# mitroitskii/crosscoder-model-diff-replication

Measured on AMD Instinct MI355X. Metric: activations/sec per train step (fwd+bwd+Adam), 2x2304->16384; % bf16 MFMA peak, higher is better.
Workload: dtype bf16; 1 GPU; crosscoder train step 2x2304->16384, batch 4096; global_batch=4096, n_models=2, d_model=2304, dict_size=16384, parallelism=latent1

## Files before the change

crosscoder-model-diff-replication_amd/csrc/gemm.hip:

```cpp
#include <mutex>

#include <hip/hip_ext.h>

#include "cc_common.h"

namespace cc {

#include "grad_tail.h"
#include "loss_tail.h"

constexpr int BM = 256, NTHR = 512;
constexpr uint32_t OOB = 0x7ffffff0u;
constexpr uint32_t MAX_RECORDS = 0x7fffffe0u;

enum Epi { EPI_F32 = 0, EPI_ENC = 1, EPI_DEC = 2, EPI_DACTS = 3, EPI_WGDEC = 4, EPI_WGENC = 5, EPI_SPLIT = 6, EPI_DLOSS = 7 };

struct GemmArgs {
  const void* A;
  const void* B;
  int64_t lda, ldb;
  int M, N, K;
  int nbm, nbn;
  void* out;
  int64_t ldo;
// ... 392 lines not shown
    const char* la = smem + (kt % NST) * STAGE;
    const char* lb = la + A_BYTES;
    if constexpr (!SPREAD) {
#pragma unroll
      for (int q = 0; q < D; ++q) dma(q, nxt, snx, pf);
    }
    if constexpr (DT == CC_BF16) {
      constexpr int KB = 1;
#pragma unroll
      for (int k0 = 0; k0 < KK; k0 += KB) {
        bf16x8 a[KB][WG::TM], b[KB][WG::TN];
#pragma unroll
        for (int u = 0; u < KB; ++u) {
#pragma unroll
          for (int j = 0; j < WG::TN; ++j) {
            const int c0 = wc * WG::WTN + j * 16;
            b[u][j] = BKC ? frag_kc_bf16<KROW>(lb, c0, k0 + u, lane) : frag_mn_bf16_at<BNT, KROW>(lb, offB[j], k0 + u);
          }
#pragma unroll
          for (int i = 0; i < WG::TM; ++i) {
            const int r0 = wr * WG::WTM + i * 16;
            a[u][i] = AKC ? frag_kc_bf16<KROW>(la, r0, k0 + u, lane) : frag_mn_bf16_at<BM, KROW>(la, offA[i], k0 + u);
          }
        }
        if (SPREAD && k0 == 0) {
#pragma unroll
          for (int q = 0; q < D; ++q) dma(q, nxt, snx, pf);
        }
#pragma unroll
        for (int u = 0; u < KB; ++u)
#pragma unroll
          for (int i = 0; i < WG::TM; ++i)
#pragma unroll
            for (int j = 0; j < WG::TN; ++j)
              acc[i][j] = __builtin_amdgcn_mfma_f32_16x16x32_bf16(b[u][j], a[u][i], acc[i][j], 0, 0, 0);
        __builtin_amdgcn_sched_group_barrier(0x100, KB * (WG::TM * (AKC ? 1 : 2) + WG::TN * (BKC ? 1 : 2)), 0);
        __builtin_amdgcn_sched_group_barrier(0x008, KB * WG::TM * WG::TN, 0);
      }
    } else {
#pragma unroll
      for (int kk = 0; kk < KK; ++kk) {
        f32x4 b[WG::TN];
#pragma unroll
        for (int j = 0; j < WG::TN; ++j) {
          const int c0 = wc * WG::WTN + j * 16;
          b[j] = BKC ? frag_kc_f32<KROW>(lb, c0, kk, lane) : frag_mn_f32_at<BNT, KROW>(lb, offB[j], kk);
        }
#pragma unroll
        for (int i = 0; i < WG::TM; ++i) {
          if (SPREAD && kk == 0) {
#pragma unroll
            for (int q = 0; q < D; ++q)
              if (q * WG::TM / D == i) dma(q, nxt, snx, pf);
          }
          const int r0 = wr * WG::WTM + i * 16;
          f32x4 a = AKC ? frag_kc_f32<KROW>(la, r0, kk, lane) : frag_mn_f32_at<BM, KROW>(la, offA[i], kk);
#pragma unroll
          for (int e = 0; e < 4; ++e)
#pragma unroll
            for (int j = 0; j < WG::TN; ++j)
              acc[i][j] = __builtin_amdgcn_mfma_f32_16x16x4f32(b[j][e], a[e], acc[i][j], 0, 0, 0);
        }
      }
    }
  }
  wait_vmcnt<0>();

  gemm_epilogue<DT, EPI, BNT>(args, acc, tm, m0, n0, wr, wc, lane, blockIdx.x * 8 + wave);
}

#include "gemm_pp.h"
#include "gemm_q4_tile.h"

constexpr int CC_WGRAD_CLOCK_WORDS = 8;
struct WgradTail {
  RedSeg red[2];
  int red_blocks[2];
  ClipArgs clip;
  unsigned* counter;
  float* tile_sum;
  uint64_t* clock;
};

template <bool AKC, bool BKC, int EPI0, int EPI1>
__global__ __launch_bounds__(NTHR, 1) void gemm_pp_dual_tail_kernel(const GemmArgs a0, const GemmArgs a1,
                                                                   const WgradTail tl) {
  __shared__ __attribute__((aligned(16))) char smem[EPI0 == EPI_WGDEC || EPI1 == EPI_WGDEC ? PP_LDS_W : PP_LDS];
  const uint64_t clk0 = __builtin_amdgcn_s_memtime(), wall0 = __builtin_amdgcn_s_memrealtime();
  {
    const int grp = threadIdx.x >> 8, t = threadIdx.x & 255;
    float(*red)[RED_COLS] = (float(*)[RED_COLS])(smem + grp * 4 * RED_COLS * sizeof(float));
    const int nred = tl.red_blocks[0] + tl.red_blocks[1];
    for (int base = 2 * (int)blockIdx.x; base < nred; base += 2 * (int)gridDim.x) {
      const int b = base + grp;
      const int role = b < tl.red_blocks[0] ? 0 : 1, rb = role ? b - tl.red_blocks[0] : b;
      if (b < nred) reduce_rows_phase1(tl.red[role], rb, t, red);
      __syncthreads();
      if (b < nred) reduce_rows_phase2<CC_BF16>(tl.red[role], rb, t, red);
      __syncthreads();
    }
  }
  const int nb0 = a0.nbm * a0.nbn;
  float* wsum_lds = (float*)(smem + PP_SLOT + 64);
  const int wave = threadIdx.x >> 6;
  for (TileLoop L(2 * nb0, a0.tile_ctr, a0.wave_sync); L.more();) {
    const int t = L.begin();
    const int tid = pp_opaque_tid();
    float w;
    if (t < nb0) w = pp_tile<AKC, BKC, EPI0>(a0, smem, t, tid);
    else w = pp_tile<AKC, BKC, EPI1>(a1, smem, t - nb0, tid);
    pp_tile_boundary();
    if ((threadIdx.x & 63) == 0) wsum_lds[wave] = w;
    L.advance(smem);
    if (!L.ctr) __syncthreads();
    if (threadIdx.x == 0) {
      float s = 0.f;
#pragma unroll
      for (int k = 0; k < 8; ++k) s += wsum_lds[k];
      tl.tile_sum[t] = s;
    }
  }
  __builtin_amdgcn_s_waitcnt(0);
  __syncthreads();
  int* last = (int*)smem;
  if (threadIdx.x == 0) {
    __builtin_amdgcn_fence(__ATOMIC_RELEASE, "agent");
    const bool is_last = atomicAdd(tl.counter, 1u) == gridDim.x - 1;
    if (is_last) __builtin_amdgcn_fence(__ATOMIC_ACQUIRE, "agent");
    *last = is_last;
  }
  __syncthreads();
  if (!*last) return;
  {
    double s[8] = {0, 0, 0, 0, 0, 0, 0, 0};
    for (int k = threadIdx.x; k < nb0; k += NTHR) s[1] += (double)tl.tile_sum[k];
    for (int k = threadIdx.x; k < nb0; k += NTHR) s[0] += (double)tl.tile_sum[nb0 + k];
    for (int k = threadIdx.x; k < tl.red_blocks[0]; k += NTHR) s[2] += (double)tl.red[0].sq_part[k];
    for (int k = threadIdx.x; k < tl.red_blocks[1]; k += NTHR) s[3] += (double)tl.red[1].sq_part[k];
    clip_finish<NTHR>(tl.clip, s, (double(*)[NTHR / 64])(smem + 64),
                      (float*)(smem + 64 + 8 * (NTHR / 64) * sizeof(double)));
  }
  if (threadIdx.x == 0) {
    atomicExch(tl.counter, 0u);
    const uint64_t clk1 = __builtin_amdgcn_s_memtime(), wall1 = __builtin_amdgcn_s_memrealtime();
    if (tl.clock) {
      tl.clock[0] += clk1 - clk0;
      tl.clock[1] += wall1 - wall0;
      tl.clock[2] += 1;
    }
  }
}

#ifndef CC_Q4_MASK
#define CC_Q4_MASK 2
#endif
#ifdef CC_DEBUG_HOOKS
static int g_pp_mask = 7, g_pp_fast = 1, g_dec_one_launch = 1, g_q4 = CC_Q4_MASK;
#define CC_DEBUG_API extern "C" __attribute__((visibility("default")))
CC_DEBUG_API void cc_debug_set_q4(int mask) { g_q4 = mask; }
CC_DEBUG_API int cc_debug_get_q4() { return CC_Q4_MASK; }
CC_DEBUG_API void cc_debug_set_pp_mask(int mask) { g_pp_mask = mask; }
CC_DEBUG_API void cc_debug_set_pp_fast(int on) { g_pp_fast = on; }
CC_DEBUG_API void cc_debug_set_dec_one_launch(int on) { g_dec_one_launch = on; }
static int g_wave_sync = 0;
static uint64_t* g_stamps = nullptr;
CC_DEBUG_API void cc_debug_set_stamps(void* buf) { g_stamps = (uint64_t*)buf; }
static int g_epi_store = 1;
CC_DEBUG_API void cc_debug_set_epi_store(int on) { g_epi_store = on; }
static void debug_epi_store(GemmArgs& a, int64_t stamp_tile0 = 0) {
  if (!g_epi_store) a.out = a.out_t = nullptr;
  if (g_stamps) a.stamps = g_stamps + stamp_tile0 * 12;
}
CC_DEBUG_API void cc_debug_set_wave_sync(int on) { g_wave_sync = on; }
static void debug_wave_sync(GemmArgs& a, hipStream_t st) {
  static uint32_t* words = nullptr;
  if (!g_wave_sync) return;
  if (!words && hipMalloc((void**)&words, 64) != hipSuccess) return;
  if (hipMemsetAsync(words, 0, 32, st) != hipSuccess) return;
  a.wave_sync = words;
  a.tile_ctr = nullptr;
}
__global__ __launch_bounds__(NTHR) void debug_spin_kernel(int64_t ticks) {
  extern __shared__ char hold[];
  const uint64_t t0 = wall_clock64();
  if (threadIdx.x == 0) hold[0] = 0;
  while (wall_clock64() - t0 < (uint64_t)ticks) __builtin_amdgcn_s_sleep(8);
}
CC_DEBUG_API int cc_debug_spin(int64_t blocks, int64_t lds_bytes, int64_t ns, void* stream) {
  if (blocks <= 0 || blocks > 4096 || lds_bytes < 0 || lds_bytes > 160 * 1024 || ns < 0 || ns > 1000000000)
    return CC_ERR_SHAPE;
  if (lds_bytes > 65536 && hipFuncSetAttribute((const void*)debug_spin_kernel,
                                               hipFuncAttributeMaxDynamicSharedMemorySize, (int)lds_bytes) != hipSuccess)
    return CC_ERR_SHAPE;
  hipLaunchKernelGGL(debug_spin_kernel, dim3((unsigned)blocks), dim3(NTHR), (unsigned)lds_bytes, (hipStream_t)stream,
                     (int64_t)(ns / 10));
  CC_LAUNCH_CHECK();
  return CC_OK;
}
CC_DEBUG_API int cc_debug_spin_ev(int64_t blocks, int64_t ns, void* stream, void* stop_event) {
  if (blocks <= 0 || blocks > 4096 || ns < 0 || ns > 1000000000) return CC_ERR_SHAPE;
  hipExtLaunchKernelGGL(debug_spin_kernel, dim3((unsigned)blocks), dim3(NTHR), 0, (hipStream_t)stream, nullptr,
                        (hipEvent_t)stop_event, 0, (int64_t)(ns / 10));
  CC_LAUNCH_CHECK();
  return CC_OK;
}
#else
constexpr int g_pp_mask = 7, g_pp_fast = 1, g_dec_one_launch = 1, g_q4 = CC_Q4_MASK;
#endif
static bool use_pp(int64_t N, bool akc, bool bkc, int dtype) {
  if (dtype != CC_BF16 || (!akc && bkc) || N % 8) return false;
  const int bit = akc && bkc ? 0 : (akc ? 1 : 2);
  return (g_pp_mask >> bit) & 1;
}
static int set_pre(GemmArgs& a, const cc_colsum_job* job) {
  if (!job) return CC_OK;
  if (!job->part || !job->out) return CC_ERR_NULL;
  if (job->rows <= 0 || job->cols <= 0 || job->ld < job->cols) return CC_ERR_SHAPE;
  a.pre = {job->part, (int)job->rows, (int)job->cols, job->ld, job->scale, job->out, nullptr, nullptr, nullptr, nullptr};
  a.pre_blocks = (int)((job->cols + RED_COLS - 1) / RED_COLS);
  return CC_OK;
}

static int set_tail(GemmArgs& a, const cc_loss_tail_job* j) {
  if (!j) return CC_OK;
  if (!j->colsum_acts || !j->tn || !j->l1_part || !j->row_part || !j->scalars || !j->counter) return CC_ERR_NULL;
  if (j->h <= 0 || j->B <= 0 || j->n <= 0 || j->ncb <= 0) return CC_ERR_SHAPE;
  a.tail = make_loss_tail_args(j->colsum_acts, j->tn, j->h, j->l1_part, j->row_part, j->ncb, j->l0_part, j->n_l0, j->ev,
                               j->ev_a, j->ev_b, j->scalars, j->l1l0_out, j->host_out, j->seq, j->B, j->n, j->counter);
  a.tail_items = a.tail.l1_wgs + a.tail.ev.nblk;
  return CC_OK;
}

extern "C" int cc_transposed_ok(int64_t B, int64_t K, int64_t h, int dtype) {
  return dtype == CC_BF16 && B % 8 == 0 && K % 8 == 0 && h % 8 == 0 && use_pp(h, true, true, dtype) &&
         use_pp(K, true, true, dtype);
}
static int pick_bn(int64_t N, bool akc, bool bkc, int dtype) {
  if (use_pp(N, akc, bkc, dtype)) return 256;
  return (!bkc && dtype == CC_BF16 && N % 288 == 0) ? 288 : 256;
}
static int64_t n_blocks(int64_t M, int64_t N, int bn) { return ((M + BM - 1) / BM) * ((N + bn - 1) / bn); }

template <int DT, bool AKC, bool BKC, int EPI, int BNT>
static int launch(GemmArgs a, hipStream_t st) {
  a.nbm = (a.M + BM - 1) / BM;
  a.nbn = (a.N + BNT - 1) / BNT;
  dim3 grid(a.nbm * a.nbn), block(NTHR);
  hipLaunchKernelGGL((gemm_kernel<DT, AKC, BKC, EPI, BNT>), grid, block, 0, st, a);
  CC_LAUNCH_CHECK();
  return CC_OK;
}

static int pp_grid(int64_t tiles) {
  static int cus = 0;
  static std::once_flag once;
  std::call_once(once, [] {
    int dev = 0, n = 0;
    if (hipGetDevice(&dev) == hipSuccess && hipDeviceGetAttribute(&n, hipDeviceAttributeMultiprocessorCount, dev) ==
                                                 hipSuccess && n > 0)
      cus = n;
    else
      cus = 256;
  });
  return (int)(tiles < cus ? tiles : cus);
}

template <bool AKC, bool BKC, int EPI>
static int launch_pp(GemmArgs a, hipStream_t st) {
#ifdef CC_DEBUG_HOOKS
  debug_epi_store(a);
#endif
  a.nbm = (a.M + BM - 1) / BM;
  a.nbn = (a.N + 255) / 256;
  if constexpr (EPI == EPI_ENC || EPI == EPI_DACTS) {
    if (g_pp_fast && a.M % BM == 0 && a.N % 256 == 0 &&
        (EPI == EPI_DACTS ? a.mask_bits != nullptr : a.flag && !a.wave_part0)) {
      if constexpr (AKC && BKC) {
        if ((g_q4 >> (EPI == EPI_ENC ? 0 : 1)) & 1 && a.K % 64 == 0 && a.K >= 128 && a.lda == a.ldb) {
          if constexpr (EPI == EPI_ENC)
            hipLaunchKernelGGL((gemm_q4_enc_kernel<true>), dim3(pp_grid(a.nbm * a.nbn)), dim3(Q4_THREADS), 0, st, a);
          else
            hipLaunchKernelGGL((gemm_q4_kernel<EPI, true>), dim3(pp_grid(a.nbm * a.nbn)), dim3(Q4_THREADS), 0, st, a);
          CC_LAUNCH_CHECK();
          return CC_OK;
        }
      }
      hipLaunchKernelGGL((gemm_pp_kernel<AKC, BKC, EPI, true>), dim3(pp_grid(a.nbm * a.nbn)), dim3(NTHR), 0, st, a);
      CC_LAUNCH_CHECK();
      return CC_OK;
    }
  }
  hipLaunchKernelGGL((gemm_pp_kernel<AKC, BKC, EPI>), dim3(pp_grid(a.nbm * a.nbn)), dim3(NTHR), 0, st, a);
  CC_LAUNCH_CHECK();
  return CC_OK;
}

template <int EPI, bool AKC, bool BKC>
static int launch_dt(int dtype, GemmArgs a, hipStream_t st) {
  if constexpr (!(!AKC && BKC)) {
    if (use_pp(a.N, AKC, BKC, dtype)) return launch_pp<AKC, BKC, EPI>(a, st);
  }
  if constexpr (!BKC) {
    if (pick_bn(a.N, AKC, BKC, dtype) == 288) return launch<CC_BF16, AKC, BKC, EPI, 288>(a, st);
  }
  if (dtype == CC_BF16) return launch<CC_BF16, AKC, BKC, EPI, 256>(a, st);
  if (dtype == CC_F32) return launch<CC_F32, AKC, BKC, EPI, 256>(a, st);
  return CC_ERR_DTYPE;
}

static bool al16(const void* p) { return ((uintptr_t)p & 15) == 0; }

static int check_gemm(const GemmArgs& a, int dtype, bool akc, bool bkc) {
  if (!a.A || !a.B) return CC_ERR_NULL;
  if (dtype != CC_BF16 && dtype != CC_F32) return CC_ERR_DTYPE;
  if (a.M <= 0 || a.N <= 0 || a.K <= 0) return CC_ERR_SHAPE;
  int epc = dtype == CC_BF16 ? 8 : 4;
  if (akc && (a.K % epc)) return CC_ERR_SHAPE;
  if (!akc && (a.M % epc)) return CC_ERR_SHAPE;
  if (bkc && (a.K % epc)) return CC_ERR_SHAPE;
  if (!bkc && (a.N % epc)) return CC_ERR_SHAPE;
  if (a.N % 4 || a.ldo % 4) return CC_ERR_SHAPE;
  if ((a.lda % epc) || (a.ldb % epc)) return CC_ERR_ALIGN;
  if (!al16(a.A) || !al16(a.B)) return CC_ERR_ALIGN;
  int es = dtype == CC_BF16 ? 2 : 4;
  uint64_t ra = akc ? (uint64_t)BM * a.lda * es : (uint64_t)a.K * a.lda * es;
  uint64_t rb = bkc ? (uint64_t)288 * a.ldb * es : (uint64_t)a.K * a.ldb * es;
  if (ra >= MAX_RECORDS || rb >= MAX_RECORDS) return CC_ERR_TOO_LARGE;
  return CC_OK;
}

}

using namespace cc;

extern "C" {

int64_t cc_col_part_rows(int64_t M) { return 2 * ((M + BM - 1) / BM); }
int64_t cc_wave_parts(int64_t M, int64_t N) { return 8 * n_blocks(M, N, 256); }
int64_t cc_wgrad_parts(int64_t h, int64_t K, int dtype) { return 8 * n_blocks(h, K, pick_bn(K, false, false, dtype)); }
int64_t cc_wgrad_tile_sums(int64_t h, int64_t K) { return 2 * n_blocks(h, K, 256) + CC_WGRAD_CLOCK_WORDS; }

int cc_gemm_f32out(const void* A, int a_layout, int64_t lda, const void* Bm, int b_layout, int64_t ldb, float* C,
                   int64_t ldc, int64_t M, int64_t N, int64_t K, int dtype, void* stream) {
  GemmArgs a = {};
  a.A = A; a.B = Bm; a.lda = lda; a.ldb = ldb; a.M = (int)M; a.N = (int)N; a.K = (int)K;
  a.out = C; a.ldo = ldc;
  if (!C) return CC_ERR_NULL;
  if (((uintptr_t)C & 15) != 0) return CC_ERR_ALIGN;
  bool akc = a_layout == CC_LAYOUT_KC, bkc = b_layout == CC_LAYOUT_KC;
  int rc = check_gemm(a, dtype, akc, bkc);
  if (rc) return rc;
  hipStream_t st = (hipStream_t)stream;
  if (akc && bkc) return launch_dt<EPI_F32, true, true>(dtype, a, st);
  if (akc && !bkc) return launch_dt<EPI_F32, true, false>(dtype, a, st);
  if (!akc && bkc) return launch_dt<EPI_F32, false, true>(dtype, a, st);
  return launch_dt<EPI_F32, false, false>(dtype, a, st);
}

int cc_encode_fwd(const void* x, const void* W_enc, const void* b_enc, const float* tn, void* acts, int apply_relu,
                  float* colsum_part, float* l1_part, float* l0_part, int64_t B, int64_t K, int64_t h, int dtype,
                  void* stream) {
  if (!acts) return CC_ERR_NULL;
  if (l1_part && !tn) return CC_ERR_NULL;
  GemmArgs a = {};
  a.A = x; a.lda = K; a.B = W_enc; a.ldb = K;
  a.M = (int)B; a.N = (int)h; a.K = (int)K;
  a.out = acts; a.ldo = h; a.bias = b_enc; a.tn = tn; a.flag = apply_relu;
  a.col_part = colsum_part; a.wave_part0 = l1_part; a.wave_part1 = l0_part;
  int rc = check_gemm(a, dtype, true, true);
  if (rc) return rc;
  return launch_dt<EPI_ENC, true, true>(dtype, a, (hipStream_t)stream);
}

int64_t cc_mask_bits_words(int64_t B, int64_t h) { return n_blocks(B, h, 256) * NTHR * 4; }

int cc_encode_fwd_t(const void* x, const void* W_enc, const void* b_enc, const float* tn, void* acts, void* acts_t,
                    int apply_relu, float* colsum_part, float* l1_part, float* l0_part, uint32_t* mask_bits,
                    uint32_t* tile_ctr, const cc_colsum_job* pre, int64_t B, int64_t K, int64_t h, int dtype,
                    void* stream) {
  if (!acts || !acts_t) return CC_ERR_NULL;
  if (l1_part && !tn) return CC_ERR_NULL;
  GemmArgs a = {};
  a.A = x; a.lda = K; a.B = W_enc; a.ldb = K;
  a.M = (int)B; a.N = (int)h; a.K = (int)K;
  a.out = acts; a.ldo = h; a.bias = b_enc; a.tn = tn; a.flag = apply_relu;
  a.col_part = colsum_part; a.wave_part0 = l1_part; a.wave_part1 = l0_part;
  a.out_t = acts_t; a.ldt = B; a.mask_bits = mask_bits; a.tile_ctr = tile_ctr;
  int rc = check_gemm(a, dtype, true, true);
  if (rc) return rc;
  if ((rc = set_pre(a, pre))) return rc;
  if (B % 8 || !al16(acts_t) || !use_pp(a.N, true, true, dtype)) return CC_ERR_SHAPE;
  if (mask_bits && !al16(mask_bits)) return CC_ERR_ALIGN;
  return launch_pp<true, true, EPI_ENC>(a, (hipStream_t)stream);
}

int cc_decode_fwd(const void* acts, const void* W_dec, const void* b_dec, float* recon_f32, void* recon_t, int64_t B,
                  int64_t h, int64_t K, int dtype, void* stream) {
  if (!recon_f32 && !recon_t) return CC_ERR_NULL;
  GemmArgs a = {};
  a.A = acts; a.lda = h; a.B = W_dec; a.ldb = K;
  a.M = (int)B; a.N = (int)K; a.K = (int)h;
  a.out = recon_t; a.out_f32 = recon_f32; a.ldo = K; a.bias = b_dec;
  int rc = check_gemm(a, dtype, true, false);
  if (rc) return rc;
  return launch_dt<EPI_DEC, true, false>(dtype, a, (hipStream_t)stream);
}

}

struct DecPlan {
  int nbn_main;
  int tail_cols;
  int nsplit, steps_per, nk;
};
static bool dec_plan(int64_t B, int64_t h, int64_t K, int dtype, DecPlan& p) {
  p = DecPlan{};
  if (dtype != CC_BF16 || K % 8 || h % 8) return false;
  const int64_t nbm = (B + BM - 1) / BM, nbn = (K + 255) / 256, tiles = nbm * nbn;
  const int64_t waves = tiles / 256;
  if (waves == 0 || tiles % 256 == 0 || (256 * waves) % nbm) return false;
  p.nbn_main = (int)(256 * waves / nbm);
  if (p.nbn_main >= nbn) return false;
  p.tail_cols = (int)(K - (int64_t)p.nbn_main * 256);
  const int64_t tail_tiles = nbm * (nbn - p.nbn_main);
  p.nk = (int)((h + 63) / 64);
  int S = (int)(256 / tail_tiles);
  if (S < 2) return false;
  if (S > p.nk) S = p.nk;
  p.steps_per = (p.nk + S - 1) / S;
  p.nsplit = (p.nk + p.steps_per - 1) / p.steps_per;
  return p.nsplit >= 2;
// ... 582 lines not shown
```

crosscoder-model-diff-replication_amd/csrc/gemm_pp.h:

```cpp

#include <type_traits>

#ifndef CC_EPI_STORE_AUX
#define CC_EPI_STORE_AUX 0
#endif
#ifndef CC_EPI_STORE_T_AUX
#define CC_EPI_STORE_T_AUX 0
#endif
#ifndef CC_WDEC_TILE_AUX
#define CC_WDEC_TILE_AUX 2
#endif
#ifndef CC_WG_OPERAND_AUX
#define CC_WG_OPERAND_AUX 0
#endif
#define PP_OPERAND_AUX(E) ((E) == EPI_WGDEC || (E) == EPI_WGENC ? CC_WG_OPERAND_AUX : 0)
#ifndef CC_EPI_STORE_T_AUX_ENC
#define CC_EPI_STORE_T_AUX_ENC CC_EPI_STORE_T_AUX
#endif
#ifndef CC_EPI_STORE_T_AUX_DLOSS
#define CC_EPI_STORE_T_AUX_DLOSS CC_EPI_STORE_T_AUX
#endif
#ifndef CC_EPI_STORE_WG_AUX
#define CC_EPI_STORE_WG_AUX 2
#endif
// ... 257 lines not shown
    const int kq = 8 * g + qq;
    const int h = pp_h(kq);
#pragma unroll
    for (int m = 0; m < 4; ++m) mn_off[m] = kq * 128 + (((2 * (m ^ h)) | (pp >> 1)) << 4) + 8 * (pp & 1);
  }

  f32x4 acc[WG::TM][WG::TN];
#pragma unroll
  for (int i = 0; i < WG::TM; ++i)
#pragma unroll
    for (int j = 0; j < WG::TN; ++j) acc[i][j] = f32x4{0.f, 0.f, 0.f, 0.f};

  if (pf) {
#pragma unroll
    for (int q = 0; q < 4; ++q) {
      const int ci = q * 8 + wave;
      __builtin_amdgcn_raw_ptr_buffer_load_lds(rw, (lds_void*)(smem + qb[3] + ci * 1024), 16,
                                               (int)piece_off(96 + ci, lane, erows, ecols, eldo), 0, 0, CC_WDEC_TILE_AUX);
    }
  }
  issue(2, 0);
  issue(3, 0);
  issue(0, 0);
  issue(1, 0);
  issue(2, 1);
  issue(3, 1);
  wait_vmcnt<6>();
  __builtin_amdgcn_s_barrier();
  if (wr == 1) __builtin_amdgcn_s_barrier();
  PP_STAMP(1);

  bf16x8 bfr[WG::TN][2];
  auto kstep = [&](auto tail, int t) {
    const char* la = smem + (t & 1) * BUF;
    const char* lb = la + TILE;
#pragma unroll
    for (int p = 0; p < 4; ++p) {
      __builtin_amdgcn_sched_barrier(0);
      const int kk = p & 1, ib = (p >> 1) * 4;
      if (p < 2) {
#pragma unroll
        for (int j = 0; j < WG::TN; ++j) {
          const int c0 = wc * WG::WTN + 16 * j;
          bfr[j][kk] = BKC ? pp_frag_kc(lb, c0, kc_off[kk]) : pp_frag_mn(lb, c0, kk, mn_off[(c0 >> 4) & 3]);
        }
      }
      bf16x8 afr[4];
#pragma unroll
      for (int ii = 0; ii < 4; ++ii) {
        const int r0 = wr * WG::WTM + 16 * (ib + ii);
        afr[ii] = AKC ? pp_frag_kc(la, r0, kc_off[kk]) : pp_frag_mn(la, r0, kk, mn_off[(r0 >> 4) & 3]);
      }
      issue_t(tail, p, p < 2 ? t + 1 : t + 2);
      wait_vmcnt<6>();
      if (p == 1) __builtin_amdgcn_s_waitcnt(0xC07F);
      __builtin_amdgcn_sched_barrier(0);
      __builtin_amdgcn_s_barrier();
      __builtin_amdgcn_sched_barrier(0);
#pragma unroll
      for (int ii = 0; ii < 4; ++ii)
#pragma unroll
        for (int j = 0; j < WG::TN; ++j)
          acc[ib + ii][j] = __builtin_amdgcn_mfma_f32_16x16x32_bf16(bfr[j][kk], afr[ii], acc[ib + ii][j], 0, 0, 0);
      __builtin_amdgcn_sched_barrier(0);
      __builtin_amdgcn_s_barrier();
    }
  };
  int t = 0;
  if (K % 64 == 0)
    for (; t < nk - 2; ++t) kstep(std::integral_constant<int, 2>{}, t);
  else
    for (; t < nk - 2; ++t) kstep(std::integral_constant<int, 0>{}, t);
  for (; t < nk; ++t) kstep(std::integral_constant<int, 1>{}, t);
  if (wr == 0) __builtin_amdgcn_s_barrier();
  PP_STAMP(2);
  const FragGeom<256> fg(args, m0, n0, wr, wc, lane);
  EpiCols<CC_BF16, 256> evec;
  if constexpr (EPI != EPI_F32 && EPI != EPI_DEC) load_epi_cols<CC_BF16, EPI, 256, FAST>(evec, args, fg, n0, tm, tn, tid);
  float cw[8][4];
  if constexpr (EPI == EPI_WGDEC) {
    if (pf) wgdec_factors<256>(args, fg, m0, n0, cw);
  }
  wait_vmcnt<0>();

  if constexpr (EPI == EPI_SPLIT) {
    float* o = (float*)args.out + ((int64_t)(tm * args.nbn + tn) * 8 + wave) * 32 * 256;
#pragma unroll
    for (int i = 0; i < WG::TM; ++i)
#pragma unroll
      for (int j = 0; j < WG::TN; ++j) *(f32x4*)(o + ((i * 4 + j) * 64 + lane) * 4) = acc[i][j];
  } else if constexpr (EPI == EPI_F32 || EPI == EPI_DEC) {
    gemm_epilogue<CC_BF16, EPI, 256>(args, acc, tm, m0, n0, wr, wc, lane, bid * 8 + wave);
  } else {
    __builtin_amdgcn_s_barrier();
    PP_STAMP(3);
    const float wsum = pp_epilogue_lds<EPI, FAST>(args, acc, smem, qb, pf, tm, m0, n0, wr, wc, lane, wave,
                                                  bid * 8 + wave, fg, evec, cw);
    PP_STAMP(4);
    PP_STAMP_WRITE(args, bid);
    return wsum;
  }
  return 0.f;
}

CC_DEV void pp_tile_boundary() {
  __builtin_amdgcn_s_waitcnt(0xC07F);
  __builtin_amdgcn_s_barrier();
}
CC_DEV int pp_opaque_tid() {
  int t = threadIdx.x;
  asm volatile("" : "+v"(t));
  return t;
}
constexpr int PP_SLOT = 2 * 256 * 128;
struct TileLoop {
  unsigned* ctr;
  unsigned* wsync;
  int x, nwx, ntx, i;
  unsigned nxt;
  CC_DEV TileLoop(int nt, unsigned* c, unsigned* ws = nullptr) : ctr(c), wsync(ws), nxt(0) {
    const int G = gridDim.x;
    x = blockIdx.x & 7;
    nwx = (G >> 3) + ((G & 7) > x);
    ntx = (nt >> 3) + ((nt & 7) > x);
    i = blockIdx.x >> 3;
  }
  CC_DEV bool more() const { return i < ntx; }
  CC_DEV int begin() {
    if (ctr && threadIdx.x == 0) nxt = atomicInc(ctr + x, (unsigned)(ntx - 1));
    return x + 8 * i;
  }
  CC_DEV void wave_wait() {
    if (threadIdx.x != 0) return;
    const unsigned k = (unsigned)(i / nwx);
    __hip_atomic_fetch_add(wsync + x, 1u, __ATOMIC_RELAXED, __HIP_MEMORY_SCOPE_AGENT);
    if (i + nwx >= ntx) return;
    const unsigned target = min((k + 1) * (unsigned)nwx, (unsigned)ntx);
    for (int it = 0; it < (1 << 16); ++it) {
      if (__hip_atomic_load(wsync + x, __ATOMIC_RELAXED, __HIP_MEMORY_SCOPE_AGENT) >= target) break;
      __builtin_amdgcn_s_sleep(1);
    }
  }
  CC_DEV void advance(char* smem, int slot_off = PP_SLOT) {
    if (!ctr) {
      if (wsync) wave_wait();
      i += nwx;
      return;
    }
    int* slot = (int*)(smem + slot_off);
    if (threadIdx.x == 0) *slot = (int)nxt;
    __syncthreads();
    i = nwx + __builtin_amdgcn_readfirstlane(*slot);
  }
};

CC_DEV bool pp_wait_ready(const GemmArgs& a, char* smem, int slot_off = PP_SLOT) {
  if (!a.wait_ctr) return true;
  int& ok = *(int*)(smem + slot_off);
  if (threadIdx.x == 0) {
    const uint64_t t0 = wall_clock64();
    int ready = 1;
    while ((int)(__hip_atomic_load(a.wait_ctr, __ATOMIC_RELAXED, __HIP_MEMORY_SCOPE_AGENT) - a.wait_target) < 0) {
      if (wall_clock64() - t0 > 100000000ull) {
        if (a.wait_err) __hip_atomic_store(a.wait_err, 1u, __ATOMIC_RELAXED, __HIP_MEMORY_SCOPE_SYSTEM);
        ready = 0;
        break;
      }
      __builtin_amdgcn_s_sleep(20);
    }
    __builtin_amdgcn_fence(__ATOMIC_ACQUIRE, "agent");
    ok = ready;
  }
  __syncthreads();
  const bool r = __builtin_amdgcn_readfirstlane(ok) != 0;
  __syncthreads();
  return r;
}

CC_DEV void pp_prologue_reduce(const GemmArgs& a, char* smem, int nwg) {
  if (a.pre_blocks <= 0) return;
  const int grp = threadIdx.x >> 8, t = threadIdx.x & 255;
  float(*red)[RED_COLS] = (float(*)[RED_COLS])(smem + grp * 4 * RED_COLS * sizeof(float));
  for (int base = 2 * (int)blockIdx.x; base < a.pre_blocks; base += 2 * nwg) {
    const int b = base + grp;
    if (b < a.pre_blocks) reduce_rows_phase1(a.pre, b, t, red);
    __syncthreads();
    if (b < a.pre_blocks) reduce_rows_phase2<CC_F32>(a.pre, b, t, red);
    __syncthreads();
  }
}

CC_DEV void pp_prologue_loss_tail(const GemmArgs& a, char* smem) {
  if (a.tail_items <= 0) return;
  const int np = min((int)gridDim.x, (a.tail_items + 1) / 2);
  if ((int)blockIdx.x >= np) return;
  const int grp = threadIdx.x >> 8, t = threadIdx.x & 255;
  float(*evred)[4] = (float(*)[4])(smem + grp * 64);
  for (int base = 2 * (int)blockIdx.x; base < a.tail_items; base += 2 * np) {
    const int item = base + grp;
    loss_tail_item(a.tail, item < a.tail_items ? item : -1, t, evred);
    __syncthreads();
  }
  int* last = (int*)(smem + 256);
  __builtin_amdgcn_s_waitcnt(0);
  __syncthreads();
  if (threadIdx.x == 0) {
    __builtin_amdgcn_fence(__ATOMIC_RELEASE, "agent");
    const bool is_last = atomicAdd(a.tail.counter, 1u) == (unsigned)(np - 1);
    if (is_last) __builtin_amdgcn_fence(__ATOMIC_ACQUIRE, "agent");
    *last = is_last;
  }
  __syncthreads();
  if (*last) {
    loss_scalars_body<LOSS_THREADS>(a.tail.scal, (double(*)[6])(smem + 512));
    if (threadIdx.x == 0) atomicExch(a.tail.counter, 0u);
  }
  __syncthreads();
}

template <bool AKC, bool BKC, int EPI, bool FAST = false>
__global__ __launch_bounds__(NTHR, 1) void gemm_pp_kernel(const GemmArgs args) {
  __shared__ __attribute__((aligned(16))) char smem[EPI == EPI_WGDEC ? PP_LDS_W : PP_LDS];
  pp_prologue_reduce(args, smem, gridDim.x);
  pp_prologue_loss_tail(args, smem);
  if (!pp_wait_ready(args, smem)) {
    for (TileLoop L(args.nbm * args.nbn, args.tile_ctr); L.more();) {
      L.begin();
      L.advance(smem);
      __syncthreads();
    }
    return;
  }
  for (TileLoop L(args.nbm * args.nbn, args.tile_ctr); L.more();) {
    pp_tile<AKC, BKC, EPI, FAST>(args, smem, L.begin(), pp_opaque_tid());
    pp_tile_boundary();
    L.advance(smem);
  }
}

template <bool AKC, bool BKC, int EPI0, int EPI1>
__global__ __launch_bounds__(NTHR, 1) void gemm_pp_dual_kernel(const GemmArgs a0, const GemmArgs a1) {
  __shared__ __attribute__((aligned(16))) char smem[EPI0 == EPI_WGDEC || EPI1 == EPI_WGDEC ? PP_LDS_W : PP_LDS];
  const int nb0 = a0.nbm * a0.nbn;
  for (TileLoop L(2 * nb0, a0.tile_ctr, a0.wave_sync); L.more();) {
    const int t = L.begin();
    const int tid = pp_opaque_tid();
    if (t < nb0) pp_tile<AKC, BKC, EPI0>(a0, smem, t, tid);
    else pp_tile<AKC, BKC, EPI1>(a1, smem, t - nb0, tid);
    pp_tile_boundary();
    L.advance(smem);
  }
}

template <bool AKC, bool BKC, int EPI, bool FAST = false>
__global__ __launch_bounds__(NTHR, 1) void gemm_pp_main_splitk_kernel(const GemmArgs a0, const GemmArgs t,
                                                                    int steps_per, int nk_total,
                                                                    int64_t split_stride) {
  __shared__ __attribute__((aligned(16))) char smem[PP_LDS];
  const int nb0 = a0.nbm * a0.nbn;
  if ((int)blockIdx.x < nb0) {
    pp_prologue_reduce(a0, smem, nb0);
    if (pp_wait_ready(a0, smem)) pp_tile<AKC, BKC, EPI, FAST>(a0, smem, blockIdx.x);
    return;
  }
  if (!pp_wait_ready(t, smem)) return;
  const int b = blockIdx.x - nb0;
  const int s = b / (t.nbm * t.nbn);
  const int tb = b - s * t.nbm * t.nbn;
  GemmArgs a = t;
  a.k_step0 = s * steps_per;
  a.k_steps = nk_total - a.k_step0 < steps_per ? nk_total - a.k_step0 : steps_per;
  a.out = (float*)t.out + s * split_stride;
  pp_tile<AKC, BKC, EPI_SPLIT>(a, smem, tb);
}

template <bool AKC, bool BKC>
__global__ __launch_bounds__(NTHR, 1) void gemm_pp_splitk_kernel(const GemmArgs args, int steps_per, int nk_total,
                                                               int64_t split_stride) {
  __shared__ __attribute__((aligned(16))) char smem[PP_LDS];
  const int s = blockIdx.x / (args.nbm * args.nbn);
  const int tb = blockIdx.x - s * args.nbm * args.nbn;
  if (!pp_wait_ready(args, smem)) return;
  GemmArgs a = args;
  a.k_step0 = s * steps_per;
  a.k_steps = nk_total - a.k_step0 < steps_per ? nk_total - a.k_step0 : steps_per;
  a.out = (float*)args.out + s * split_stride;
  pp_tile<AKC, BKC, EPI_SPLIT>(a, smem, tb);
}
```

crosscoder-model-diff-replication_amd/csrc/gemm_q4_tile.h:

```cpp
#pragma once
#include "gemm_q4.h"

constexpr int Q4_SLOT = Q4_LDS;
constexpr int Q4_LDS_ALL = Q4_LDS + 64;
CC_DEV int opaque_v(int v) {
  asm volatile("" : "+v"(v));
  return v;
}

CC_DEV void q4_prologue_reduce(const GemmArgs& a, char* smem) {
  if (a.pre_blocks <= 0) return;
  float(*red)[RED_COLS] = (float(*)[RED_COLS])smem;
  for (int b = blockIdx.x; b < a.pre_blocks; b += gridDim.x) {
    reduce_rows_phase1(a.pre, b, threadIdx.x, red);
    __syncthreads();
    reduce_rows_phase2<CC_F32>(a.pre, b, threadIdx.x, red);
    __syncthreads();
  }
}
CC_DEV void q4_prologue_loss_tail(const GemmArgs& a, char* smem) {
  if (a.tail_items <= 0) return;
  const int np = min((int)gridDim.x, a.tail_items);
  if ((int)blockIdx.x >= np) return;
  float(*evred)[4] = (float(*)[4])smem;
  for (int item = blockIdx.x; item < a.tail_items; item += np) {
    loss_tail_item(a.tail, item, threadIdx.x, evred);
    __syncthreads();
  }
  int* last = (int*)(smem + 256);
  __builtin_amdgcn_s_waitcnt(0);
  __syncthreads();
  if (threadIdx.x == 0) {
    __builtin_amdgcn_fence(__ATOMIC_RELEASE, "agent");
    const bool is_last = atomicAdd(a.tail.counter, 1u) == (unsigned)(np - 1);
    if (is_last) __builtin_amdgcn_fence(__ATOMIC_ACQUIRE, "agent");
    *last = is_last;
  }
  __syncthreads();
  if (*last) {
    loss_scalars_body<LOSS_THREADS>(a.tail.scal, (double(*)[6])(smem + 512));
    if (threadIdx.x == 0) atomicExch(a.tail.counter, 0u);
  }
  __syncthreads();
}

template <int EPI, bool FAST>
CC_DEV void q4_tile(const GemmArgs& args, char* smem, int bid, int tid, float (&wsum)[2]) {
  static_assert(EPI == EPI_ENC || EPI == EPI_DACTS || EPI == EPI_WGDEC || EPI == EPI_WGENC, "q4 epilogues");
  int lane = tid & 63;
  const int wave = __builtin_amdgcn_readfirstlane(tid >> 6);
  const int wr = wave >> 1, wc = wave & 1;
  int tm, tn;
  tile_of_block(bid, args.nbm, args.nbn, tm, tn);
  const int m0 = tm * BM, n0 = tn * 256;
  const int M = args.M, N = args.N;
  EpiCols<CC_BF16, 256> ev[2];
#pragma unroll
  for (int h = 0; h < 2; ++h)
    load_epi_cols<CC_BF16, EPI, 256, FAST>(ev[h], args, FragGeom<256>(args, m0, n0, wr, 2 * wc + h, lane), n0, tm, tn,
                                           (4 * wr + 2 * wc + h) * 64 + lane);
  f32x4 acc[8][8];
  q4_kloop(acc, (const char*)args.A + (int64_t)m0 * args.lda * 2, (const char*)args.B + (int64_t)n0 * args.ldb * 2,
           args.lda, (uint64_t)(M - m0) * args.lda * 2, (uint64_t)(N - n0) * args.ldb * 2, args.K / 64, smem, lane, wave);
  lane = opaque_v(lane);
  const FragGeom<256> fg[2] = {FragGeom<256>(args, m0, n0, wr, 2 * wc, lane),
                               FragGeom<256>(args, m0, n0, wr, 2 * wc + 1, lane)};
  __syncthreads();
  const int rows = M - m0, cols = N - n0, ldo = (int)args.ldo;
  const int qb[4] = {0, Q4_IMG, 2 * Q4_IMG, 3 * Q4_IMG};
  const void* in = (EPI == EPI_DACTS && !FAST) ? args.mask_src
                                               : (EPI == EPI_WGDEC && args.scale0 != 0.f ? args.w_src : nullptr);
  if (in) {
    const __amdgpu_buffer_rsrc_t rin = tile_rsrc(in, args.ldo, m0, n0, args.M, args.N, 2);
#pragma unroll
    for (int q = 0; q < 32; ++q) {
      const int ci = q * 4 + wave;
      __builtin_amdgcn_raw_ptr_buffer_load_lds(rin, (lds_void*)(smem + qb[ci >> 5] + (ci & 31) * 1024), 16,
                                               (int)piece_off(ci, lane, rows, cols, ldo), 0, 0,
                                               EPI == EPI_WGDEC ? CC_WDEC_TILE_AUX : 0);
    }
  }
  float cw[2][8][4];
  if constexpr (EPI == EPI_WGDEC) {
    if (in) {
#pragma unroll
      for (int h = 0; h < 2; ++h) wgdec_factors<256>(args, fg[h], m0, n0, cw[h]);
    }
  }
  if (in) {
    wait_vmcnt<0>();
    __builtin_amdgcn_s_barrier();
  }
#pragma unroll
  for (int h = 0; h < 2; ++h) {
    f32x4 ah[8][4];
#pragma unroll
    for (int i = 0; i < 8; ++i)
#pragma unroll
      for (int j = 0; j < 4; ++j) ah[i][j] = acc[i][4 * h + j];
    const LdsIO io(smem, qb, wr, 2 * wc + h, lane);
    wsum[h] = epilogue_core<CC_BF16, EPI, 256, FAST>(args, ah, fg[h], io, tm, m0, n0, wr, lane,
                                                     bid * 8 + 4 * wr + 2 * wc + h, ev[h], cw[h]);
  }
  __syncthreads();
  if (args.out) {
    const __amdgpu_buffer_rsrc_t rout = tile_rsrc(args.out, args.ldo, m0, n0, args.M, args.N, 2);
#pragma unroll
    for (int q = 0; q < 32; ++q) {
      const int ci = q * 4 + wave;
      const bf16x8 v = *(const bf16x8*)(smem + qb[ci >> 5] + (ci & 31) * 1024 + lane * 16);
      __builtin_amdgcn_raw_buffer_store_b128(__builtin_bit_cast(u32x4, v), rout, (int)piece_off(ci, lane, rows, cols, ldo),
                                             0, EPI == EPI_WGDEC || EPI == EPI_WGENC ? CC_EPI_STORE_WG_AUX : CC_EPI_STORE_AUX);
    }
  }
  if (args.out_t)
    pp_store_transposed<EPI == EPI_ENC ? CC_EPI_STORE_T_AUX_ENC : CC_EPI_STORE_T_AUX, 4>(args, smem, qb, m0, n0, rows,
                                                                                       cols, lane, wave);
}

template <int EPI, bool FAST>
CC_DEV void q4_kernel_body(const GemmArgs& args) {
  __shared__ __attribute__((aligned(16))) char smem[Q4_LDS_ALL];
  q4_prologue_reduce(args, smem);
  q4_prologue_loss_tail(args, smem);
  if (!pp_wait_ready(args, smem, Q4_SLOT)) {
    for (TileLoop L(args.nbm * args.nbn, args.tile_ctr); L.more();) {
      L.begin();
      L.advance(smem, Q4_SLOT);
      __syncthreads();
    }
    return;
  }
  for (TileLoop L(args.nbm * args.nbn, args.tile_ctr); L.more();) {
    float w[2];
    q4_tile<EPI, FAST>(args, smem, L.begin(), pp_opaque_tid(), w);
    pp_tile_boundary();
    L.advance(smem, Q4_SLOT);
  }
}
template <int EPI, bool FAST>
__global__ __launch_bounds__(Q4_THREADS, 1) void gemm_q4_kernel(const GemmArgs args) {
  q4_kernel_body<EPI, FAST>(args);
}
#ifndef CC_Q4_ENC_VGPRS
#define CC_Q4_ENC_VGPRS 160
#endif
template <bool FAST>
__global__ __launch_bounds__(Q4_THREADS, 1) __attribute__((amdgpu_num_vgpr(CC_Q4_ENC_VGPRS))) void gemm_q4_enc_kernel(
    const GemmArgs args) {
  q4_kernel_body<EPI_ENC, FAST>(args);
}
```

Before: 1.645 million activations/s.

## Enable q4 encoder kernel with late epilogue-column loads and deferred tile claim

Turns on the q4 MFMA path for the encoder GEMM by default, but only when a transposed output is requested. The encoder q4 kernel now loads epilogue columns after the K-loop instead of before it, which frees registers during the main loop. It also claims the next tile atomically after the epilogue instead of at the start of the tile. The VGPR cap rises to 176 to fit the new schedule. The risk is that the late loads now sit exposed before the epilogue, and that the encoder path changes behaviour when it is selected.

```diff
diff --git a/crosscoder-model-diff-replication_amd/csrc/gemm.hip b/crosscoder-model-diff-replication_amd/csrc/gemm.hip
--- a/crosscoder-model-diff-replication_amd/csrc/gemm.hip
+++ b/crosscoder-model-diff-replication_amd/csrc/gemm.hip
@@ -568,7 +568,7 @@
 }
 
 #ifndef CC_Q4_MASK
-#define CC_Q4_MASK 2
+#define CC_Q4_MASK 3
 #endif
 #ifdef CC_DEBUG_HOOKS
 static int g_pp_mask = 7, g_pp_fast = 1, g_dec_one_launch = 1, g_q4 = CC_Q4_MASK;
@@ -692,7 +692,8 @@
     if (g_pp_fast && a.M % BM == 0 && a.N % 256 == 0 &&
         (EPI == EPI_DACTS ? a.mask_bits != nullptr : a.flag && !a.wave_part0)) {
       if constexpr (AKC && BKC) {
-        if ((g_q4 >> (EPI == EPI_ENC ? 0 : 1)) & 1 && a.K % 64 == 0 && a.K >= 128 && a.lda == a.ldb) {
+        if ((g_q4 >> (EPI == EPI_ENC ? 0 : 1)) & 1 && a.K % 64 == 0 && a.K >= 128 && a.lda == a.ldb &&
+            (EPI != EPI_ENC || a.out_t)) {
           if constexpr (EPI == EPI_ENC)
             hipLaunchKernelGGL((gemm_q4_enc_kernel<true>), dim3(pp_grid(a.nbm * a.nbn)), dim3(Q4_THREADS), 0, st, a);
           else
diff --git a/crosscoder-model-diff-replication_amd/csrc/gemm_pp.h b/crosscoder-model-diff-replication_amd/csrc/gemm_pp.h
--- a/crosscoder-model-diff-replication_amd/csrc/gemm_pp.h
+++ b/crosscoder-model-diff-replication_amd/csrc/gemm_pp.h
@@ -433,6 +433,22 @@
     __syncthreads();
     i = nwx + __builtin_amdgcn_readfirstlane(*slot);
   }
+  CC_DEV int tile() const { return x + 8 * i; }
+  CC_DEV void claim(int tid) {
+    unsigned v = 0;
+    if (ctr && tid == 0) v = atomicInc(ctr + x, (unsigned)(ntx - 1));
+    nxt = v;
+  }
+  CC_DEV void advance_claimed(char* smem, int slot_off, int tid) {
+    if (!ctr) {
+      i += nwx;
+      return;
+    }
+    int* slot = (int*)(smem + slot_off);
+    if (tid == 0) *slot = (int)nxt;
+    __syncthreads();
+    i = nwx + __builtin_amdgcn_readfirstlane(*slot);
+  }
 };
 
 CC_DEV bool pp_wait_ready(const GemmArgs& a, char* smem, int slot_off = PP_SLOT) {
diff --git a/crosscoder-model-diff-replication_amd/csrc/gemm_q4_tile.h b/crosscoder-model-diff-replication_amd/csrc/gemm_q4_tile.h
--- a/crosscoder-model-diff-replication_amd/csrc/gemm_q4_tile.h
+++ b/crosscoder-model-diff-replication_amd/csrc/gemm_q4_tile.h
@@ -6,6 +6,10 @@
 CC_DEV int opaque_v(int v) {
   asm volatile("" : "+v"(v));
   return v;
+}
+CC_DEV float* opaque_s(float* p) {
+  asm volatile("" : "+s"(p));
+  return p;
 }
 
 CC_DEV void q4_prologue_reduce(const GemmArgs& a, char* smem) {
@@ -44,8 +48,14 @@
   __syncthreads();
 }
 
-template <int EPI, bool FAST>
-CC_DEV void q4_tile(const GemmArgs& args, char* smem, int bid, int tid, float (&wsum)[2]) {
+CC_DEV int q4_rebuilt_tid(int wave) {
+  int l;
+  asm volatile("v_mbcnt_lo_u32_b32 %0, -1, 0\n\tv_mbcnt_hi_u32_b32 %0, -1, %0" : "=&v"(l));
+  return wave * 64 + l;
+}
+
+template <int EPI, bool FAST, bool LATE = false>
+CC_DEV void q4_tile(const GemmArgs& args, char* smem, int bid, int tid, float (&wsum)[2], TileLoop* L = nullptr) {
   static_assert(EPI == EPI_ENC || EPI == EPI_DACTS || EPI == EPI_WGDEC || EPI == EPI_WGENC, "q4 epilogues");
   int lane = tid & 63;
   const int wave = __builtin_amdgcn_readfirstlane(tid >> 6);
@@ -55,16 +65,27 @@
   const int m0 = tm * BM, n0 = tn * 256;
   const int M = args.M, N = args.N;
   EpiCols<CC_BF16, 256> ev[2];
+  if constexpr (!LATE) {
 #pragma unroll
-  for (int h = 0; h < 2; ++h)
-    load_epi_cols<CC_BF16, EPI, 256, FAST>(ev[h], args, FragGeom<256>(args, m0, n0, wr, 2 * wc + h, lane), n0, tm, tn,
-                                           (4 * wr + 2 * wc + h) * 64 + lane);
+    for (int h = 0; h < 2; ++h)
+      load_epi_cols<CC_BF16, EPI, 256, FAST>(ev[h], args, FragGeom<256>(args, m0, n0, wr, 2 * wc + h, lane), n0, tm,
+                                             tn, (4 * wr + 2 * wc + h) * 64 + lane);
+  }
   f32x4 acc[8][8];
   q4_kloop(acc, (const char*)args.A + (int64_t)m0 * args.lda * 2, (const char*)args.B + (int64_t)n0 * args.ldb * 2,
            args.lda, (uint64_t)(M - m0) * args.lda * 2, (uint64_t)(N - n0) * args.ldb * 2, args.K / 64, smem, lane, wave);
-  lane = opaque_v(lane);
+  if constexpr (LATE) {
+    lane = q4_rebuilt_tid(wave) & 63;
+  } else {
+    lane = opaque_v(lane);
+  }
   const FragGeom<256> fg[2] = {FragGeom<256>(args, m0, n0, wr, 2 * wc, lane),
                                FragGeom<256>(args, m0, n0, wr, 2 * wc + 1, lane)};
+  if constexpr (LATE) {
+#pragma unroll
+    for (int h = 0; h < 2; ++h)
+      load_epi_cols<CC_BF16, EPI, 256, FAST>(ev[h], args, fg[h], n0, tm, tn, (4 * wr + 2 * wc + h) * 64 + lane);
+  }
   __syncthreads();
   const int rows = M - m0, cols = N - n0, ldo = (int)args.ldo;
   const int qb[4] = {0, Q4_IMG, 2 * Q4_IMG, 3 * Q4_IMG};
@@ -91,6 +112,13 @@
     wait_vmcnt<0>();
     __builtin_amdgcn_s_barrier();
   }
+  GemmArgs la;
+  const GemmArgs* ea = &args;
+  if constexpr (LATE) {
+    la = args;
+    la.col_part = opaque_s(la.col_part);
+    ea = &la;
+  }
 #pragma unroll
   for (int h = 0; h < 2; ++h) {
     f32x4 ah[8][4];
@@ -99,9 +127,10 @@
 #pragma unroll
       for (int j = 0; j < 4; ++j) ah[i][j] = acc[i][4 * h + j];
     const LdsIO io(smem, qb, wr, 2 * wc + h, lane);
-    wsum[h] = epilogue_core<CC_BF16, EPI, 256, FAST>(args, ah, fg[h], io, tm, m0, n0, wr, lane,
+    wsum[h] = epilogue_core<CC_BF16, EPI, 256, FAST>(*ea, ah, fg[h], io, tm, m0, n0, wr, lane,
                                                      bid * 8 + 4 * wr + 2 * wc + h, ev[h], cw[h]);
   }
+  if constexpr (LATE) L->claim(q4_rebuilt_tid(wave));
   __syncthreads();
   if (args.out) {
     const __amdgpu_buffer_rsrc_t rout = tile_rsrc(args.out, args.ldo, m0, n0, args.M, args.N, 2);
@@ -118,7 +147,7 @@
                                                                                        cols, lane, wave);
 }
 
-template <int EPI, bool FAST>
+template <int EPI, bool FAST, bool LATE = false>
 CC_DEV void q4_kernel_body(const GemmArgs& args) {
   __shared__ __attribute__((aligned(16))) char smem[Q4_LDS_ALL];
   q4_prologue_reduce(args, smem);
@@ -131,11 +160,21 @@
     }
     return;
   }
-  for (TileLoop L(args.nbm * args.nbn, args.tile_ctr); L.more();) {
-    float w[2];
-    q4_tile<EPI, FAST>(args, smem, L.begin(), pp_opaque_tid(), w);
-    pp_tile_boundary();
-    L.advance(smem, Q4_SLOT);
+  if constexpr (LATE) {
+    const int wave = __builtin_amdgcn_readfirstlane((int)threadIdx.x >> 6);
+    for (TileLoop L(args.nbm * args.nbn, args.tile_ctr); L.more();) {
+      float w[2];
+      q4_tile<EPI, FAST, true>(args, smem, L.tile(), q4_rebuilt_tid(wave), w, &L);
+      pp_tile_boundary();
+      L.advance_claimed(smem, Q4_SLOT, q4_rebuilt_tid(wave));
+    }
+  } else {
+    for (TileLoop L(args.nbm * args.nbn, args.tile_ctr); L.more();) {
+      float w[2];
+      q4_tile<EPI, FAST>(args, smem, L.begin(), pp_opaque_tid(), w);
+      pp_tile_boundary();
+      L.advance(smem, Q4_SLOT);
+    }
   }
 }
 template <int EPI, bool FAST>
@@ -143,10 +182,10 @@
   q4_kernel_body<EPI, FAST>(args);
 }
 #ifndef CC_Q4_ENC_VGPRS
-#define CC_Q4_ENC_VGPRS 160
+#define CC_Q4_ENC_VGPRS 176
 #endif
 template <bool FAST>
 __global__ __launch_bounds__(Q4_THREADS, 1) __attribute__((amdgpu_num_vgpr(CC_Q4_ENC_VGPRS))) void gemm_q4_enc_kernel(
     const GemmArgs args) {
-  q4_kernel_body<EPI_ENC, FAST>(args);
+  q4_kernel_body<EPI_ENC, FAST, true>(args);
 }
```

Measured after the change: 1.652 million activations/s (median of 6 runs). About the same (+0.4%).
